# Plonky3/Plonky3-recursion

Measured on AMD Instinct MI355X. Metric: prove_next_layer ms + Poseidon2 perms/s, KoalaBear 2^20-row circuit, 1/8 GPU, lower is better.
Workload: dtype u32 Montgomery (31-bit prime field, degree-4 extension); Poseidon2 hashing as exact integers in f64; 1 GPU; prove_next_layer (verifier-circuit run on the device + prove_all_tables) of the synthetic koala-bear 2^20-row recursion layer: tables const/public/alu/poseidon2/recompose, FRI blowup 4, arity<=4, 54 queries, 15-bit PoW; circuit inputs + NextLayerPrepCache resident in HBM; field=koala-bear, log_height=20, independent_proofs=1, proof_bytes=612900, parallelism=1 independent proofs, one per GPU, no data-path collective

## Files before the change

### plonky3_recursion_amd/csrc/kernels_ntt2.hip.h

```cpp
#pragma once
#include "kernels_ntt.hip.h"

namespace p3r {

constexpr int kNtt2LogTile = 13;
constexpr int kNtt2Lanes = 512;

template <class PP>
constexpr uint32_t ntt2_root_mont(int log_r, uint32_t idx, bool inverse) {
  uint32_t g = pow_mod(PP::GEN, ((uint64_t)PP::P - 1) >> log_r, PP::P);
  if (inverse) g = pow_mod(g, (uint64_t)PP::P - 2, PP::P);
  const uint64_t w = pow_mod(g, idx, PP::P);
  return (uint32_t)((w << 32) % PP::P);
}

template <class PP, int LOG_R, int S, int ML, bool INV>
struct Ntt2LastTw {
  uint32_t v[4][8];
  constexpr Ntt2LastTw() : v() {
    for (int u = 0; u < ML; ++u)
      for (int jj = 0; jj < ((1 << ML) >> (u + 1)); ++jj) v[u][jj] = ntt2_root_mont<PP>(LOG_R, (uint32_t)jj << (S + u), INV);
  }
};

template <class PP>
__device__ __forceinline__ void ntt2_bfly(Fp<PP>& p, Fp<PP>& c, uint32_t tw) {
  using F = Fp<PP>;
  const F s = p + c;
  c = F::raw(F::reduce64((uint64_t)(p.v + (PP::P - c.v)) * tw));
  p = s;
}
template <class PP>
__device__ __forceinline__ void ntt2_bfly_one(Fp<PP>& p, Fp<PP>& c) {
  const Fp<PP> s = p + c, d = p - c;
  p = s;
  c = d;
}

template <class PP, int LOG_R, int S, int ML, bool LAST, bool INV = false, class TW = const uint32_t*>
__device__ __forceinline__ void ntt2_stages(Fp<PP>* x, TW tws, uint32_t low) {
  constexpr int M = 1 << ML;
  constexpr int LQ = LOG_R - S - ML;
  static_assert(!LAST || LQ == 0, "the last group ends the transform");
  constexpr Ntt2LastTw<PP, LOG_R, S, ML, INV> kLast{};
#pragma unroll
  for (int u = 0; u < ML; ++u) {
    const int half = M >> (u + 1);
#pragma unroll
    for (int jj = 0; jj < M / 2; ++jj) {
      if (jj < half) {
        uint32_t tw = 0;
        const bool one = LAST && jj == 0;
        if constexpr (!LAST) tw = tws[(low << (S + u)) + ((uint32_t)jj << (LQ + S + u))];
#pragma unroll
        for (int it = 0; it < 16 / M; ++it) {
#pragma unroll
          for (int blk = 0; blk < M; blk += 2 * half) {
            Fp<PP>& p = x[it * M + blk + jj];
            Fp<PP>& c = x[it * M + blk + jj + half];
            if (LAST) {
              if (one) ntt2_bfly_one<PP>(p, c);
              else ntt2_bfly<PP>(p, c, kLast.v[u][jj]);
            } else {
              ntt2_bfly<PP>(p, c, tw);
            }
          }
        }
      }
    }
  }
}

template <int LOG_R>
__device__ __forceinline__ uint32_t ntt2_line_pos(uint32_t t, uint32_t r) {
  constexpr uint32_t LINE = (1u << LOG_R) + (1u << (LOG_R > 4 ? LOG_R - 4 : 0));
  return t * LINE + r + (r >> 4);
}

template <class PP, int LOG_R, int S>
__device__ __forceinline__ void ntt2_line_middle(uint32_t* tile, const uint32_t* tws, Fp<PP>* x, uint32_t tid) {
  using F = Fp<PP>;
  constexpr uint32_t R = 1u << LOG_R;
  constexpr int LQ = LOG_R - S - 4;
  const uint32_t it = tid & ((R / 16) - 1), t = tid >> (LOG_R - 4);
  const uint32_t low = it & ((1u << LQ) - 1), high = it >> LQ;
  const uint32_t r0 = (high << (LQ + 4)) | low;
#pragma unroll
  for (int j = 0; j < 16; ++j) x[j] = F::raw(tile[ntt2_line_pos<LOG_R>(t, r0 + ((uint32_t)j << LQ))]);
  ntt2_stages<PP, LOG_R, S, 4, false>(x, tws, low);
#pragma unroll
  for (int j = 0; j < 16; ++j) tile[ntt2_line_pos<LOG_R>(t, r0 + ((uint32_t)j << LQ))] = x[j].v;
  __syncthreads();
}

struct NttLineJob {
  uint32_t* data;
  const uint32_t* tw;
  uint32_t block0;
  uint32_t log_r;
};

constexpr uint32_t ntt2_line_tile_words(int log_r, int log_tile) {
  return ((1u << log_r) + (1u << (log_r - 4))) << (log_tile - log_r);
}

template <class PP, int LOG_R, int LOG_TILE>
__device__ __forceinline__ void ntt2_line_body(const NttLineJob& job, uint32_t local, uint32_t* tile, uint32_t* tws) {
  using F = Fp<PP>;
  static_assert(LOG_R >= 5 && LOG_R <= LOG_TILE && LOG_TILE <= 13, "line length");
  constexpr uint32_t R = 1u << LOG_R;
  constexpr uint32_t LANES = 1u << (LOG_TILE - 4);
  constexpr int G = (LOG_R + 3) / 4;
  constexpr int ML_LAST = LOG_R - 4 * (G - 1);
  const gptr<uint32_t> data = as_global(job.data) + ((size_t)local << LOG_TILE);
  const gptr<const uint32_t> twg = as_global(job.tw);
  const uint32_t tid = threadIdx.x;
  for (uint32_t i = tid; i < R / 2; i += LANES) tws[i] = twg[i];
  F x[16];
  {
    constexpr int LQ = LOG_R - 4;
    const uint32_t b = tid & ((1u << LQ) - 1), t = tid >> LQ;
    const gptr<uint32_t> src = data + (t << LOG_R) + b;
#pragma unroll
    for (int j = 0; j < 16; ++j) x[j] = F::raw(src[(uint32_t)j << LQ]);
    __syncthreads();
    ntt2_stages<PP, LOG_R, 0, 4, LOG_R == 4>(x, tws, b);
#pragma unroll
    for (int j = 0; j < 16; ++j) tile[ntt2_line_pos<LOG_R>(t, b + ((uint32_t)j << LQ))] = x[j].v;
  }
  __syncthreads();
  if constexpr (G >= 3) ntt2_line_middle<PP, LOG_R, 4>(tile, tws, x, tid);
  if constexpr (G >= 4) ntt2_line_middle<PP, LOG_R, 8>(tile, tws, x, tid);
  {
    constexpr int S = 4 * (G - 1);
    const uint32_t it = tid & ((R / 16) - 1), t = tid >> (LOG_R - 4);
    const uint32_t r0 = it << 4;
#pragma unroll
    for (int j = 0; j < 16; ++j) x[j] = F::raw(tile[ntt2_line_pos<LOG_R>(t, r0 + j)]);
    ntt2_stages<PP, LOG_R, S, ML_LAST, true>(x, (const uint32_t*)nullptr, 0);
#pragma unroll
    for (int j = 0; j < 16; ++j) tile[ntt2_line_pos<LOG_R>(t, r0 + j)] = x[j].v;
  }
  __syncthreads();
#pragma unroll
  for (int j = 0; j < 16; ++j) {
    const uint32_t cell = tid + (uint32_t)j * LANES;
    data[cell] = tile[ntt2_line_pos<LOG_R>(cell >> LOG_R, cell & (R - 1))];
  }
}

template <class PP, int LOG_R, int LOG_TILE = kNtt2LogTile>
__global__ void __launch_bounds__(1 << (LOG_TILE - 4)) k_ntt_fwd_line(const NttLineJob* __restrict__ jobs, int n_jobs) {
  __shared__ uint32_t tile[ntt2_line_tile_words(LOG_R, LOG_TILE)];
  __shared__ uint32_t tws[(1u << LOG_R) / 2];
  const int jb = find_job(jobs, n_jobs);
  ntt2_line_body<PP, LOG_R, LOG_TILE>(jobs[jb], blockIdx.x - jobs[jb].block0, tile, tws);
}

template <class PP>
__global__ void __launch_bounds__(256) k_ntt_fwd_line_mixed(const NttLineJob* __restrict__ jobs, int n_jobs) {
  __shared__ uint32_t tile[ntt2_line_tile_words(12, 12)];
  __shared__ uint32_t tws[(1u << 12) / 2];
  const int jb = find_job(jobs, n_jobs);
  const NttLineJob& job = jobs[jb];
  const uint32_t local = blockIdx.x - job.block0;
  switch (job.log_r) {
    case 5: ntt2_line_body<PP, 5, 12>(job, local, tile, tws); break;
    case 6: ntt2_line_body<PP, 6, 12>(job, local, tile, tws); break;
    case 7: ntt2_line_body<PP, 7, 12>(job, local, tile, tws); break;
    case 8: ntt2_line_body<PP, 8, 12>(job, local, tile, tws); break;
    case 9: ntt2_line_body<PP, 9, 12>(job, local, tile, tws); break;
    case 10: ntt2_line_body<PP, 10, 12>(job, local, tile, tws); break;
    case 11: ntt2_line_body<PP, 11, 12>(job, local, tile, tws); break;
    default: ntt2_line_body<PP, 12, 12>(job, local, tile, tws); break;
  }
}

enum { NTT2_FWD = 0, NTT2_INV1 = 1, NTT2_INV2 = 2 };
struct NttColJob {
  const uint32_t* in;
  uint32_t* out;
  const uint32_t* tw;
  const uint32_t* tw4_lo;
  const uint32_t* tw4_hi;
  const uint32_t* pre_a;
  const uint32_t* pre_b;
  uint64_t in_col_stride, out_col_stride, out_coset_stride;
  int log_n2, log_cosets;
  int log_r;
  uint32_t scale;
  uint32_t block0;
  uint32_t xcd_map;
};

constexpr uint32_t ntt2_col_tile_words(int log_r, int log_tile) {
  return (1u << log_r) * ((1u << (log_tile - log_r)) + 1) + ((1u << log_r) >> 5) + 2;
}

template <class PP, int LOG_R, int MODE, int LOG_TILE>
__device__ __forceinline__ void ntt2_col_body(const NttColJob& a, uint32_t local, uint32_t* tile, uint32_t* tws) {
  using F = Fp<PP>;
  static_assert(LOG_R >= 5 && LOG_R <= 12, "sub-transform size");
  static_assert(LOG_TILE == 13 || LOG_TILE == 14, "tile size");
  constexpr bool INV = MODE != NTT2_FWD;
  constexpr uint32_t R = 1u << LOG_R;
  constexpr int LOG_T = LOG_TILE - LOG_R;
  constexpr uint32_t T = 1u << LOG_T;
  constexpr int ITEMS = 1 << (LOG_TILE - kNtt2LogTile);
  constexpr int G = (LOG_R + 3) / 4;
  constexpr int ML_LAST = LOG_R - 4 * (G - 1);
  const int log_gx = a.log_n2 - LOG_T;
  uint32_t bx, bz, by;
  if (a.xcd_map) {
    const uint32_t xcd = local & 7, slot = local >> 3;
    bz = slot & ((1u << a.log_cosets) - 1);
    const uint32_t tile_lin = ((slot >> a.log_cosets) << 3) | xcd;
    bx = tile_lin & ((1u << log_gx) - 1);
    by = tile_lin >> log_gx;
  } else {
    bx = local & ((1u << log_gx) - 1);
    bz = (local >> log_gx) & ((1u << a.log_cosets) - 1);
    by = local >> (log_gx + a.log_cosets);
  }
  const uint32_t tid = threadIdx.x;
  const gptr<const uint32_t> twg = as_global(a.tw);
  for (uint32_t i = tid; i < R / 2; i += kNtt2Lanes) tws[i] = twg[i];
  F x[16];
#pragma unroll
  for (int item = 0; item < ITEMS; ++item) {
    const uint32_t e = tid + (uint32_t)item * kNtt2Lanes;
    const uint32_t t = e & (T - 1), it = e >> LOG_T;
    const uint32_t n2 = (bx << LOG_T) + t;
    constexpr int LQ = LOG_R - 4;
    const gptr<const uint32_t> src = as_global(a.in) + (size_t)by * a.in_col_stride + n2;
    if constexpr (MODE == NTT2_FWD) {
      const gptr<const uint32_t> pa = as_global(a.pre_a) + ((size_t)bz << LOG_R);
#pragma unroll
      for (int j = 0; j < 16; ++j) {
        const uint32_t n1 = it + ((uint32_t)j << LQ);
        x[j] = F::raw(src[(size_t)n1 << a.log_n2]) * F::raw(pa[n1]);
      }
    } else {
#pragma unroll
      for (int j = 0; j < 16; ++j) x[j] = F::raw(src[(size_t)(it + ((uint32_t)j << LQ)) << a.log_n2]);
    }
    if (item == 0) __syncthreads();
    ntt2_stages<PP, LOG_R, 0, 4, false, INV>(x, tws, it);
#pragma unroll
    for (int j = 0; j < 16; ++j) tile[lds_addr(it + ((uint32_t)j << LQ), t, T)] = x[j].v;
  }
  __syncthreads();
  if constexpr (G >= 3) {
#pragma unroll
    for (int item = 0; item < ITEMS; ++item) {
      const uint32_t e = tid + (uint32_t)item * kNtt2Lanes;
      const uint32_t t = e & (T - 1), it = e >> LOG_T;
      constexpr int S = 4;
      constexpr int LQ = LOG_R - S - 4;
      const uint32_t low = it & ((1u << LQ) - 1), high = it >> LQ;
      const uint32_t r0 = (high << (LQ + 4)) | low;
#pragma unroll
      for (int j = 0; j < 16; ++j) x[j] = F::raw(tile[lds_addr(r0 + ((uint32_t)j << LQ), t, T)]);
      ntt2_stages<PP, LOG_R, S, 4, false, INV>(x, tws, low);
#pragma unroll
      for (int j = 0; j < 16; ++j) tile[lds_addr(r0 + ((uint32_t)j << LQ), t, T)] = x[j].v;
    }
    __syncthreads();
  }
  constexpr int S_LAST = 4 * (G - 1);
  const gptr<uint32_t> dst = as_global(a.out) + (size_t)by * a.out_col_stride + (size_t)bz * a.out_coset_stride;
#pragma unroll
  for (int item = 0; item < ITEMS; ++item) {
    const uint32_t e = tid + (uint32_t)item * kNtt2Lanes;
    const uint32_t t = e & (T - 1), it = e >> LOG_T;
    const uint32_t n2 = (bx << LOG_T) + t;
    const uint32_t r0 = it << 4;
#pragma unroll
    for (int j = 0; j < 16; ++j) x[j] = F::raw(tile[lds_addr(r0 + j, t, T)]);
    ntt2_stages<PP, LOG_R, S_LAST, ML_LAST, true, INV>(x, (const uint32_t*)nullptr, 0);
    if constexpr (MODE == NTT2_FWD) {
      const gptr<const uint32_t> lo = as_global(a.tw4_lo), hi = as_global(a.tw4_hi);
      auto w_pow = [&](uint32_t e) {
        const uint32_t v = F::reduce64_lazy((uint64_t)hi[e >> 10] * lo[e & 1023]);
        return F::raw(min(v, v - PP::P));
      };
      const F pb = F::raw(as_global(a.pre_b)[((size_t)bz << a.log_n2) + n2]);
      const F g = w_pow(n2 << (LOG_R - 4));
      const F g2 = g * g, g4 = g2 * g2;
      F head[4];
      head[0] = w_pow(bit_reverse(it, LOG_R - 4) * n2) * pb;
      head[1] = head[0] * g;
      head[2] = head[0] * g2;
      head[3] = head[1] * g2;
#pragma unroll
      for (int m = 0; m < 4; ++m) {
#pragma unroll
        for (int q = 0; q < 4; ++q) {
          constexpr int kRev4[16] = {0, 8, 4, 12, 2, 10, 6, 14, 1, 9, 5, 13, 3, 11, 7, 15};
          const int j = kRev4[4 * m + q];
          dst[((size_t)(r0 + j) << a.log_n2) + n2] = (x[j] * head[q]).v;
          if (m < 3) head[q] = head[q] * g4;
        }
      }
    } else if constexpr (MODE == NTT2_INV2) {
      const F sc = F::raw(a.scale);
#pragma unroll
      for (int j = 0; j < 16; ++j) {
        const uint32_t k1 = bit_reverse(r0 + j, LOG_R);
        dst[((size_t)k1 << a.log_n2) + n2] = (x[j] * sc).v;
      }
    } else {
#pragma unroll
      for (int j = 0; j < 16; ++j) tile[lds_addr(r0 + j, t, T)] = x[j].v;
    }
  }
  if constexpr (MODE == NTT2_INV1) {
    __syncthreads();
    const gptr<const uint32_t> lo = as_global(a.tw4_lo), hi = as_global(a.tw4_hi);
#pragma unroll
    for (int j = 0; j < 16 * ITEMS; ++j) {
      const uint32_t e = tid + (uint32_t)j * kNtt2Lanes;
      const uint32_t k1 = e & (R - 1), tt = e >> LOG_R;
      const uint32_t col = (bx << LOG_T) + tt;
      const uint32_t xk = k1 * col;
      const F tw = F::raw(F::reduce64_lazy((uint64_t)hi[xk >> 10] * lo[xk & 1023]));
      const F v = F::raw(tile[lds_addr(bit_reverse(k1, LOG_R), tt, T)]);
      dst[((size_t)col << LOG_R) + k1] = (v * tw).v;
    }
  }
}

template <class PP, int LOG_R, int MODE, int LOG_TILE = kNtt2LogTile>
__global__ void __launch_bounds__(kNtt2Lanes, LOG_TILE == 13 ? 8 : 4) k_ntt_col(const NttColJob* __restrict__ jobs, int n_jobs) {
  __shared__ uint32_t tile[ntt2_col_tile_words(LOG_R, LOG_TILE)];
  __shared__ uint32_t tws[(1u << LOG_R) / 2];
  const int jb = find_job(jobs, n_jobs);
  ntt2_col_body<PP, LOG_R, MODE, LOG_TILE>(jobs[jb], blockIdx.x - jobs[jb].block0, tile, tws);
}

constexpr uint32_t kNtt2MixedMaxBlocks = 2048;
template <class PP, int MODE>
__global__ void __launch_bounds__(kNtt2Lanes) k_ntt_col_mixed(const NttColJob* __restrict__ jobs, int n_jobs) {
  __shared__ uint32_t tile[ntt2_col_tile_words(12, 13)];
  __shared__ uint32_t tws[(1u << 12) / 2];
  const int jb = find_job(jobs, n_jobs);
  const NttColJob& a = jobs[jb];
  const uint32_t local = blockIdx.x - a.block0;
  switch (a.log_r) {
    case 5: ntt2_col_body<PP, 5, MODE, 13>(a, local, tile, tws); break;
    case 6: ntt2_col_body<PP, 6, MODE, 13>(a, local, tile, tws); break;
    case 7: ntt2_col_body<PP, 7, MODE, 13>(a, local, tile, tws); break;
    case 8: ntt2_col_body<PP, 8, MODE, 13>(a, local, tile, tws); break;
    case 9: ntt2_col_body<PP, 9, MODE, 13>(a, local, tile, tws); break;
    case 10: ntt2_col_body<PP, 10, MODE, 13>(a, local, tile, tws); break;
    case 11: ntt2_col_body<PP, 11, MODE, 13>(a, local, tile, tws); break;
    default: ntt2_col_body<PP, 12, MODE, 13>(a, local, tile, tws); break;
  }
}

}
```

Baseline: 26.23 ms.

## Use radix-4 butterflies with paired-product REDC in NTT stage groups

Replaces pairs of radix-2 DIF stages with a radix-4 step that computes the outputs as dot products of two terms, each followed by a single Montgomery reduction. This cuts the number of modular reductions per stage pair. It adds a small shared-memory table of w^3 twiddles, whose granularity K3 is picked at compile time so that occupancy is not reduced. The cost is extra twiddle loads and larger LDS allocations, and the new butterfly math carries correctness risk.

```diff
diff --git a/plonky3_recursion_amd/csrc/kernels_ntt2.hip.h b/plonky3_recursion_amd/csrc/kernels_ntt2.hip.h
--- a/plonky3_recursion_amd/csrc/kernels_ntt2.hip.h
+++ b/plonky3_recursion_amd/csrc/kernels_ntt2.hip.h
@@ -1,73 +1,18 @@
 #pragma once
 #include "kernels_ntt.hip.h"
+#include "ntt2_butterfly.h"
 
 namespace p3r {
 
 constexpr int kNtt2LogTile = 13;
 constexpr int kNtt2Lanes = 512;
 
-template <class PP>
-constexpr uint32_t ntt2_root_mont(int log_r, uint32_t idx, bool inverse) {
-  uint32_t g = pow_mod(PP::GEN, ((uint64_t)PP::P - 1) >> log_r, PP::P);
-  if (inverse) g = pow_mod(g, (uint64_t)PP::P - 2, PP::P);
-  const uint64_t w = pow_mod(g, idx, PP::P);
-  return (uint32_t)((w << 32) % PP::P);
-}
-
-template <class PP, int LOG_R, int S, int ML, bool INV>
-struct Ntt2LastTw {
-  uint32_t v[4][8];
-  constexpr Ntt2LastTw() : v() {
-    for (int u = 0; u < ML; ++u)
-      for (int jj = 0; jj < ((1 << ML) >> (u + 1)); ++jj) v[u][jj] = ntt2_root_mont<PP>(LOG_R, (uint32_t)jj << (S + u), INV);
-  }
-};
-
-template <class PP>
-__device__ __forceinline__ void ntt2_bfly(Fp<PP>& p, Fp<PP>& c, uint32_t tw) {
-  using F = Fp<PP>;
-  const F s = p + c;
-  c = F::raw(F::reduce64((uint64_t)(p.v + (PP::P - c.v)) * tw));
-  p = s;
-}
-template <class PP>
-__device__ __forceinline__ void ntt2_bfly_one(Fp<PP>& p, Fp<PP>& c) {
-  const Fp<PP> s = p + c, d = p - c;
-  p = s;
-  c = d;
-}
-
-template <class PP, int LOG_R, int S, int ML, bool LAST, bool INV = false, class TW = const uint32_t*>
-__device__ __forceinline__ void ntt2_stages(Fp<PP>* x, TW tws, uint32_t low) {
-  constexpr int M = 1 << ML;
-  constexpr int LQ = LOG_R - S - ML;
-  static_assert(!LAST || LQ == 0, "the last group ends the transform");
-  constexpr Ntt2LastTw<PP, LOG_R, S, ML, INV> kLast{};
-#pragma unroll
-  for (int u = 0; u < ML; ++u) {
-    const int half = M >> (u + 1);
-#pragma unroll
-    for (int jj = 0; jj < M / 2; ++jj) {
-      if (jj < half) {
-        uint32_t tw = 0;
-        const bool one = LAST && jj == 0;
-        if constexpr (!LAST) tw = tws[(low << (S + u)) + ((uint32_t)jj << (LQ + S + u))];
-#pragma unroll
-        for (int it = 0; it < 16 / M; ++it) {
-#pragma unroll
-          for (int blk = 0; blk < M; blk += 2 * half) {
-            Fp<PP>& p = x[it * M + blk + jj];
-            Fp<PP>& c = x[it * M + blk + jj + half];
-            if (LAST) {
-              if (one) ntt2_bfly_one<PP>(p, c);
-              else ntt2_bfly<PP>(p, c, kLast.v[u][jj]);
-            } else {
-              ntt2_bfly<PP>(p, c, tw);
-            }
-          }
-        }
-      }
-    }
+template <class PP, int LOG_R, int K3, uint32_t LANES>
+__device__ __forceinline__ void ntt2_load_twiddles(uint32_t* tws, gptr<const uint32_t> twg, uint32_t tid) {
+  constexpr uint32_t R = 1u << LOG_R;
+  for (uint32_t i = tid; i < R / 2; i += LANES) tws[i] = twg[i];
+  if constexpr (K3 < LOG_R - 1) {
+    for (uint32_t i = tid; i < ((R / 2) >> K3); i += LANES) tws[R / 2 + i] = ntt2_tw3_entry<PP, LOG_R, K3>(twg, i);
   }
 }
 
@@ -77,7 +22,7 @@
   return t * LINE + r + (r >> 4);
 }
 
-template <class PP, int LOG_R, int S>
+template <class PP, int LOG_R, int S, int K3>
 __device__ __forceinline__ void ntt2_line_middle(uint32_t* tile, const uint32_t* tws, Fp<PP>* x, uint32_t tid) {
   using F = Fp<PP>;
   constexpr uint32_t R = 1u << LOG_R;
@@ -87,7 +32,7 @@
   const uint32_t r0 = (high << (LQ + 4)) | low;
 #pragma unroll
   for (int j = 0; j < 16; ++j) x[j] = F::raw(tile[ntt2_line_pos<LOG_R>(t, r0 + ((uint32_t)j << LQ))]);
-  ntt2_stages<PP, LOG_R, S, 4, false>(x, tws, low);
+  ntt2_stages<PP, LOG_R, S, 4, false, false, K3>(x, tws, low);
 #pragma unroll
   for (int j = 0; j < 16; ++j) tile[ntt2_line_pos<LOG_R>(t, r0 + ((uint32_t)j << LQ))] = x[j].v;
   __syncthreads();
@@ -104,7 +49,10 @@
   return ((1u << log_r) + (1u << (log_r - 4))) << (log_tile - log_r);
 }
 
-template <class PP, int LOG_R, int LOG_TILE>
+constexpr int ntt2_line_k3(int log_r, int log_tile) {
+  return ntt2_k3(log_r, ntt2_line_tile_words(log_r, log_tile), 1u << (log_tile - 4));
+}
+template <class PP, int LOG_R, int LOG_TILE, int K3 = ntt2_line_k3(LOG_R, LOG_TILE)>
 __device__ __forceinline__ void ntt2_line_body(const NttLineJob& job, uint32_t local, uint32_t* tile, uint32_t* tws) {
   using F = Fp<PP>;
   static_assert(LOG_R >= 5 && LOG_R <= LOG_TILE && LOG_TILE <= 13, "line length");
@@ -115,7 +63,7 @@
   const gptr<uint32_t> data = as_global(job.data) + ((size_t)local << LOG_TILE);
   const gptr<const uint32_t> twg = as_global(job.tw);
   const uint32_t tid = threadIdx.x;
-  for (uint32_t i = tid; i < R / 2; i += LANES) tws[i] = twg[i];
+  ntt2_load_twiddles<PP, LOG_R, K3, LANES>(tws, twg, tid);
   F x[16];
   {
     constexpr int LQ = LOG_R - 4;
@@ -124,13 +72,13 @@
 #pragma unroll
     for (int j = 0; j < 16; ++j) x[j] = F::raw(src[(uint32_t)j << LQ]);
     __syncthreads();
-    ntt2_stages<PP, LOG_R, 0, 4, LOG_R == 4>(x, tws, b);
+    ntt2_stages<PP, LOG_R, 0, 4, false, false, K3>(x, tws, b);
 #pragma unroll
     for (int j = 0; j < 16; ++j) tile[ntt2_line_pos<LOG_R>(t, b + ((uint32_t)j << LQ))] = x[j].v;
   }
   __syncthreads();
-  if constexpr (G >= 3) ntt2_line_middle<PP, LOG_R, 4>(tile, tws, x, tid);
-  if constexpr (G >= 4) ntt2_line_middle<PP, LOG_R, 8>(tile, tws, x, tid);
+  if constexpr (G >= 3) ntt2_line_middle<PP, LOG_R, 4, K3>(tile, tws, x, tid);
+  if constexpr (G >= 4) ntt2_line_middle<PP, LOG_R, 8, K3>(tile, tws, x, tid);
   {
     constexpr int S = 4 * (G - 1);
     const uint32_t it = tid & ((R / 16) - 1), t = tid >> (LOG_R - 4);
@@ -152,7 +100,7 @@
 template <class PP, int LOG_R, int LOG_TILE = kNtt2LogTile>
 __global__ void __launch_bounds__(1 << (LOG_TILE - 4)) k_ntt_fwd_line(const NttLineJob* __restrict__ jobs, int n_jobs) {
   __shared__ uint32_t tile[ntt2_line_tile_words(LOG_R, LOG_TILE)];
-  __shared__ uint32_t tws[(1u << LOG_R) / 2];
+  __shared__ uint32_t tws[ntt2_tw_words(LOG_R, ntt2_line_k3(LOG_R, LOG_TILE))];
   const int jb = find_job(jobs, n_jobs);
   ntt2_line_body<PP, LOG_R, LOG_TILE>(jobs[jb], blockIdx.x - jobs[jb].block0, tile, tws);
 }
@@ -160,7 +108,7 @@
 template <class PP>
 __global__ void __launch_bounds__(256) k_ntt_fwd_line_mixed(const NttLineJob* __restrict__ jobs, int n_jobs) {
   __shared__ uint32_t tile[ntt2_line_tile_words(12, 12)];
-  __shared__ uint32_t tws[(1u << 12) / 2];
+  __shared__ uint32_t tws[ntt2_tw_words(12, ntt2_line_k3(12, 12))];
   const int jb = find_job(jobs, n_jobs);
   const NttLineJob& job = jobs[jb];
   const uint32_t local = blockIdx.x - job.block0;
@@ -174,6 +122,7 @@
     case 11: ntt2_line_body<PP, 11, 12>(job, local, tile, tws); break;
     default: ntt2_line_body<PP, 12, 12>(job, local, tile, tws); break;
   }
+  static_assert(ntt2_tw_words(11, ntt2_line_k3(11, 12)) <= ntt2_tw_words(12, ntt2_line_k3(12, 12)), "twiddle table of the mixed launch");
 }
 
 enum { NTT2_FWD = 0, NTT2_INV1 = 1, NTT2_INV2 = 2 };
@@ -197,7 +146,8 @@
   return (1u << log_r) * ((1u << (log_tile - log_r)) + 1) + ((1u << log_r) >> 5) + 2;
 }
 
-template <class PP, int LOG_R, int MODE, int LOG_TILE>
+constexpr int ntt2_col_k3(int log_r, int log_tile) { return ntt2_k3(log_r, ntt2_col_tile_words(log_r, log_tile), kNtt2Lanes); }
+template <class PP, int LOG_R, int MODE, int LOG_TILE, int K3 = ntt2_col_k3(LOG_R, LOG_TILE)>
 __device__ __forceinline__ void ntt2_col_body(const NttColJob& a, uint32_t local, uint32_t* tile, uint32_t* tws) {
   using F = Fp<PP>;
   static_assert(LOG_R >= 5 && LOG_R <= 12, "sub-transform size");
@@ -224,7 +174,7 @@
   }
   const uint32_t tid = threadIdx.x;
   const gptr<const uint32_t> twg = as_global(a.tw);
-  for (uint32_t i = tid; i < R / 2; i += kNtt2Lanes) tws[i] = twg[i];
+  ntt2_load_twiddles<PP, LOG_R, K3, kNtt2Lanes>(tws, twg, tid);
   F x[16];
 #pragma unroll
   for (int item = 0; item < ITEMS; ++item) {
@@ -245,7 +195,7 @@
       for (int j = 0; j < 16; ++j) x[j] = F::raw(src[(size_t)(it + ((uint32_t)j << LQ)) << a.log_n2]);
     }
     if (item == 0) __syncthreads();
-    ntt2_stages<PP, LOG_R, 0, 4, false, INV>(x, tws, it);
+    ntt2_stages<PP, LOG_R, 0, 4, false, INV, K3>(x, tws, it);
 #pragma unroll
     for (int j = 0; j < 16; ++j) tile[lds_addr(it + ((uint32_t)j << LQ), t, T)] = x[j].v;
   }
@@ -261,7 +211,7 @@
       const uint32_t r0 = (high << (LQ + 4)) | low;
 #pragma unroll
       for (int j = 0; j < 16; ++j) x[j] = F::raw(tile[lds_addr(r0 + ((uint32_t)j << LQ), t, T)]);
-      ntt2_stages<PP, LOG_R, S, 4, false, INV>(x, tws, low);
+      ntt2_stages<PP, LOG_R, S, 4, false, INV, K3>(x, tws, low);
 #pragma unroll
       for (int j = 0; j < 16; ++j) tile[lds_addr(r0 + ((uint32_t)j << LQ), t, T)] = x[j].v;
     }
@@ -333,7 +283,7 @@
 template <class PP, int LOG_R, int MODE, int LOG_TILE = kNtt2LogTile>
 __global__ void __launch_bounds__(kNtt2Lanes, LOG_TILE == 13 ? 8 : 4) k_ntt_col(const NttColJob* __restrict__ jobs, int n_jobs) {
   __shared__ uint32_t tile[ntt2_col_tile_words(LOG_R, LOG_TILE)];
-  __shared__ uint32_t tws[(1u << LOG_R) / 2];
+  __shared__ uint32_t tws[ntt2_tw_words(LOG_R, ntt2_col_k3(LOG_R, LOG_TILE))];
   const int jb = find_job(jobs, n_jobs);
   ntt2_col_body<PP, LOG_R, MODE, LOG_TILE>(jobs[jb], blockIdx.x - jobs[jb].block0, tile, tws);
 }
@@ -342,7 +292,7 @@
 template <class PP, int MODE>
 __global__ void __launch_bounds__(kNtt2Lanes) k_ntt_col_mixed(const NttColJob* __restrict__ jobs, int n_jobs) {
   __shared__ uint32_t tile[ntt2_col_tile_words(12, 13)];
-  __shared__ uint32_t tws[(1u << 12) / 2];
+  __shared__ uint32_t tws[ntt2_tw_words(12, ntt2_col_k3(12, 13))];
   const int jb = find_job(jobs, n_jobs);
   const NttColJob& a = jobs[jb];
   const uint32_t local = blockIdx.x - a.block0;
diff --git a/plonky3_recursion_amd/csrc/ntt2_butterfly.h b/plonky3_recursion_amd/csrc/ntt2_butterfly.h
--- /dev/null
+++ b/plonky3_recursion_amd/csrc/ntt2_butterfly.h
@@ -0,0 +1,169 @@
+#pragma once
+#include "field.h"
+
+namespace p3r {
+
+template <class PP>
+constexpr uint32_t ntt2_root_mont(int log_r, uint32_t idx, bool inverse) {
+  uint32_t g = pow_mod(PP::GEN, ((uint64_t)PP::P - 1) >> log_r, PP::P);
+  if (inverse) g = pow_mod(g, (uint64_t)PP::P - 2, PP::P);
+  const uint64_t w = pow_mod(g, idx, PP::P);
+  return (uint32_t)((w << 32) % PP::P);
+}
+
+template <class PP, int LOG_R, int SH, bool INV>
+struct Ntt2LastTw {
+  uint32_t w1[8], iw1[4], w2[4], w3[4], niw3[4];
+  constexpr Ntt2LastTw() : w1(), iw1(), w2(), w3(), niw3() {
+    constexpr uint32_t R = 1u << LOG_R;
+    for (uint32_t jj = 0; jj < 8; ++jj) w1[jj] = ntt2_root_mont<PP>(LOG_R, (jj << SH) & (R - 1), INV);
+    for (uint32_t jj = 0; jj < 4; ++jj) {
+      const uint32_t k = (jj << SH) & (R - 1);
+      iw1[jj] = ntt2_root_mont<PP>(LOG_R, (k + R / 4) & (R - 1), INV);
+      w2[jj] = ntt2_root_mont<PP>(LOG_R, (2 * k) & (R - 1), INV);
+      w3[jj] = ntt2_root_mont<PP>(LOG_R, (3 * k) & (R - 1), INV);
+      niw3[jj] = ntt2_root_mont<PP>(LOG_R, (3 * k + 3 * (R / 4)) & (R - 1), INV);
+    }
+  }
+};
+
+template <class PP>
+P3R_HD void ntt2_bfly(Fp<PP>& p, Fp<PP>& c, uint32_t tw) {
+  using F = Fp<PP>;
+  const F s = p + c;
+  c = F::raw(F::reduce64((uint64_t)(p.v + (PP::P - c.v)) * tw));
+  p = s;
+}
+template <class PP>
+P3R_HD void ntt2_bfly_one(Fp<PP>& p, Fp<PP>& c) {
+  const Fp<PP> s = p + c, d = p - c;
+  p = s;
+  c = d;
+}
+
+template <class PP>
+P3R_HD Fp<PP> ntt2_dot2(Fp<PP> x, uint32_t w1, Fp<PP> y, uint32_t w2) {
+  static_assert(2 * (uint64_t)(PP::P - 1) * (PP::P - 1) < ((uint64_t)PP::P << 32), "a paired product stays inside REDC's input range");
+  return Fp<PP>::raw(Fp<PP>::reduce64((uint64_t)x.v * w1 + (uint64_t)y.v * w2));
+}
+
+template <class PP>
+P3R_HD void ntt2_bfly4(Fp<PP>& a, Fp<PP>& b, Fp<PP>& c, Fp<PP>& d, uint32_t W1, uint32_t IW1, uint32_t W2, uint32_t nW2,
+                       uint32_t W3, uint32_t nIW3) {
+  const Fp<PP> t0 = a + c, t1 = b + d, u0 = a - c, u1 = b - d;
+  a = t0 + t1;
+  b = ntt2_dot2<PP>(t0, W2, t1, nW2);
+  c = ntt2_dot2<PP>(u0, W1, u1, IW1);
+  d = ntt2_dot2<PP>(u0, W3, u1, nIW3);
+}
+template <class PP>
+P3R_HD void ntt2_bfly4_one(Fp<PP>& a, Fp<PP>& b, Fp<PP>& c, Fp<PP>& d, uint32_t I) {
+  ntt2_bfly_one<PP>(a, c);
+  ntt2_bfly<PP>(b, d, I);
+  ntt2_bfly_one<PP>(a, b);
+  ntt2_bfly_one<PP>(c, d);
+}
+
+constexpr int kNtt2NoTw3 = 32;
+constexpr uint32_t ntt2_tw_words(int log_r, int k3) {
+  return (1u << log_r) / 2 + (k3 >= log_r - 1 ? 0u : ((1u << log_r) / 2) >> k3);
+}
+constexpr int ntt2_k3(int log_r, uint32_t tile_words, uint32_t lanes) {
+  const uint32_t cap = 32 / (lanes / 64);
+  const uint32_t base = (160u * 1024) / (4 * (tile_words + ntt2_tw_words(log_r, kNtt2NoTw3)));
+  const uint32_t want = base < cap ? base : cap;
+  for (int k3 = 0; k3 < log_r - 1; k3 += 2) {
+    const uint32_t got = (160u * 1024) / (4 * (tile_words + ntt2_tw_words(log_r, k3)));
+    if ((got < cap ? got : cap) >= want) return k3;
+  }
+  return kNtt2NoTw3;
+}
+
+template <class PP, int LOG_R, int K3, class TW>
+P3R_HD uint32_t ntt2_tw3_entry(TW tw, uint32_t i) {
+  constexpr uint32_t R = 1u << LOG_R;
+  const uint32_t e = (3 * (i << K3)) & (R - 1);
+  const uint32_t v = tw[e & (R / 2 - 1)];
+  return e < R / 2 ? v : PP::P - v;
+}
+
+template <class PP, int LOG_R, int S, int ML, int U, bool LAST, bool INV, class TW>
+P3R_HD void ntt2_stage2(Fp<PP>* x, TW tws, uint32_t low) {
+  constexpr int M = 1 << ML;
+  constexpr int LQ = LOG_R - S - ML;
+  constexpr int half = M >> (U + 1);
+  constexpr Ntt2LastTw<PP, LOG_R, S + U, INV> kLast{};
+#pragma unroll
+  for (int jj = 0; jj < half; ++jj) {
+    uint32_t tw = 0;
+    if constexpr (LAST) tw = kLast.w1[jj];
+    else tw = tws[(low << (S + U)) + ((uint32_t)jj << (LQ + S + U))];
+#pragma unroll
+    for (int it = 0; it < 16 / M; ++it) {
+#pragma unroll
+      for (int blk = 0; blk < M; blk += 2 * half) {
+        Fp<PP>& p = x[it * M + blk + jj];
+        Fp<PP>& c = x[it * M + blk + jj + half];
+        if (LAST && jj == 0) ntt2_bfly_one<PP>(p, c);
+        else ntt2_bfly<PP>(p, c, tw);
+      }
+    }
+  }
+}
+
+template <class PP, int LOG_R, int S, int ML, int U, bool LAST, bool INV, int K3, class TW>
+P3R_HD void ntt2_step4(Fp<PP>* x, TW tws, uint32_t low) {
+  constexpr int M = 1 << ML;
+  constexpr int LQ = LOG_R - S - ML;
+  constexpr int SH = S + U;
+  constexpr int QH = M >> (U + 2);
+  constexpr uint32_t R = 1u << LOG_R;
+  constexpr Ntt2LastTw<PP, LOG_R, SH, INV> kLast{};
+#pragma unroll
+  for (int jj = 0; jj < QH; ++jj) {
+    uint32_t W1 = 0, IW1 = 0, W2 = 0, W3 = 0, nIW3 = 0;
+    if constexpr (LAST) {
+      W1 = kLast.w1[jj], IW1 = kLast.iw1[jj], W2 = kLast.w2[jj], W3 = kLast.w3[jj], nIW3 = kLast.niw3[jj];
+    } else {
+      static_assert(LAST || SH >= K3, "the w^3j table is too coarse for this stage");
+      const uint32_t k = (low << SH) + ((uint32_t)jj << (LQ + SH));
+      W1 = tws[k];
+      IW1 = tws[k + R / 4];
+      W2 = tws[2 * k];
+      W3 = tws[R / 2 + (k >> K3)];
+      nIW3 = tws[R / 2 + ((k + R / 4) >> K3)];
+    }
+    const uint32_t nW2 = PP::P - W2;
+#pragma unroll
+    for (int it = 0; it < 16 / M; ++it) {
+#pragma unroll
+      for (int blk = 0; blk < M; blk += 4 * QH) {
+        Fp<PP>* y = x + it * M + blk + jj;
+        if (LAST && jj == 0) ntt2_bfly4_one<PP>(y[0], y[QH], y[2 * QH], y[3 * QH], IW1);
+        else ntt2_bfly4<PP>(y[0], y[QH], y[2 * QH], y[3 * QH], W1, IW1, W2, nW2, W3, nIW3);
+      }
+    }
+  }
+}
+
+template <class PP, int LOG_R, int S, int ML, bool LAST, bool INV = false, int K3 = kNtt2NoTw3, class TW = const uint32_t*>
+P3R_HD void ntt2_stages(Fp<PP>* x, TW tws, uint32_t low) {
+  static_assert(!LAST || LOG_R - S - ML == 0, "the last group ends the transform");
+  static_assert(ML >= 1 && ML <= 4, "stages per group");
+  constexpr bool R4_0 = ML >= 2 && (LAST || S >= K3);
+  constexpr bool R4_2 = ML >= 4 && (LAST || S + 2 >= K3);
+  if constexpr (R4_0) {
+    ntt2_step4<PP, LOG_R, S, ML, 0, LAST, INV, K3>(x, tws, low);
+  } else {
+    ntt2_stage2<PP, LOG_R, S, ML, 0, LAST, INV>(x, tws, low);
+    if constexpr (ML >= 2) ntt2_stage2<PP, LOG_R, S, ML, 1, LAST, INV>(x, tws, low);
+  }
+  if constexpr (R4_2) {
+    ntt2_step4<PP, LOG_R, S, ML, 2, LAST, INV, K3>(x, tws, low);
+  } else {
+    if constexpr (ML >= 3) ntt2_stage2<PP, LOG_R, S, ML, 2, LAST, INV>(x, tws, low);
+    if constexpr (ML >= 4) ntt2_stage2<PP, LOG_R, S, ML, 3, LAST, INV>(x, tws, low);
+  }
+}
+
+}
```

New measurement: 26.00 ms (median of 6 runs). No clear change (-0.9%).
